# Intsights/PySubstringSearch

Measured on AMD Instinct MI355X. Metric: queries/sec (batched) + index-build GB/s on 512MB chunk, 1/2/4/8 GPU, higher is better.
Workload: dtype u64

## Files before the change

### include/pss.h

```cpp
#ifndef PSS_H
#define PSS_H

#include <stddef.h>
#include <stdint.h>

#ifdef __cplusplus
extern "C" {
#endif

#define PSS_OK 0
#define PSS_EINVAL (-1)
#define PSS_ENOMEM (-2)
#define PSS_EIO (-3)
#define PSS_ETOOBIG (-4)
#define PSS_EDEVICE (-5)
#define PSS_EFORMAT (-6)

typedef struct pss_writer pss_writer;
typedef struct pss_reader pss_reader;
typedef struct pss_result pss_result;


int pss_device_count(void);

// ... 233 lines not shown
    int (*send)(const void *buf, size_t count, int datatype, int peer, void *comm, void *stream);
    int (*recv)(void *buf, size_t count, int datatype, int peer, void *comm, void *stream);
    int (*all_gather)(const void *sendbuf, void *recvbuf, size_t sendcount, int datatype, void *comm, void *stream);
    const char *(*get_error_string)(int result);
} pss_rccl_api;
int pss_rccl_inject(const pss_rccl_api *api);
int pss_comm_adopt(void *nccl_comm, int32_t world, int32_t rank, int32_t device, pss_comm **out);

int pss_merge_packed(uint32_t world, uint64_t nq, const uint64_t *const *counts, const uint64_t *const *offsets,
                     const uint8_t *const *bytes, const uint64_t *num_entries, const uint64_t *num_bytes,
                     uint64_t *out_counts, uint64_t *out_offsets, uint8_t *out_bytes);
int pss_merge_packed_device(int32_t device, uint32_t world, uint64_t nq, const void *const *d_counts,
                            const void *const *d_starts, const void *const *d_bytes, const uint64_t *num_entries,
                            const uint64_t *num_bytes, void *d_out_counts, void *d_out_offsets, void *d_out_bytes);
int pss_reader_last_stats(const pss_reader *r, pss_search_stats *stats);
int pss_reader_close(pss_reader *r);

uint64_t pss_result_num_queries(const pss_result *res);
uint64_t pss_result_num_entries(const pss_result *res);
const uint64_t *pss_result_query_counts(const pss_result *res);
const uint64_t *pss_result_offsets(const pss_result *res);
const uint8_t *pss_result_bytes(const pss_result *res);
void pss_result_free(pss_result *res);


#define PSS_CORPUS_LINES 0
#define PSS_CORPUS_WORDS 1
#define PSS_CORPUS_RUNS 2
#define PSS_CORPUS_PERIODIC 3
#define PSS_CORPUS_REPEAT_LINE 4
// ... 10 lines not shown
```

### pysubstringsearch_amd/__init__.py

```python
import ctypes
import os
import typing

from . import _ffi
from ._ffi import lib as _lib

try:
    from . import _pssglue
except ImportError:
    _pssglue = None

__all__ = ['Writer', 'Reader', 'PackedResult', 'IdResult', 'DeviceResult', 'device_count', 'default_devices', 'release_workspace', 'workspace_bytes',
           'glob_parse', 'glob_escape', 'icase_variants']


def device_count() -> int:
    return _lib.pss_device_count()


def release_workspace() -> None:
    _ffi.check(_lib.pss_release_workspace())


def workspace_bytes(device: int = 0) -> int:
# ... 755 lines not shown
        import numpy as np
        nq = len(patterns)
        blob, offs = _pack_queries(patterns)
        counts = np.zeros(max(nq, 1), dtype=np.uint64)
        _ffi.check(_lib.pss_reader_count_batch(self._handle(), blob, offs.ctypes.data, nq, counts.ctypes.data))
        return [int(c) for c in counts[:nq]]

    def search_batch_raw(self, patterns: typing.Sequence[bytes]):
        return self._search_batch(patterns, False)

    def last_stats(self) -> dict:
        st = _ffi.SearchStats()
        _ffi.check(_lib.pss_reader_last_stats(self._handle(), ctypes.byref(st)))
        return st.as_dict()

    def search(self, substring: str) -> typing.List[str]:
        return self._search_batch([_utf8(substring, 'substring')], True)[0]

    def search_multiple(self, substrings: typing.List[str]) -> typing.List[str]:
        return self._search_batch([_utf8(s, 'substring') for s in substrings], True)[0]

    def close(self) -> None:
        if self._h:
            h, self._h = self._h, ctypes.c_void_p()
            _lib.pss_reader_close(h)

    def __enter__(self):
        return self

    def __exit__(self, *exc):
# ... 8 lines not shown
```

### pysubstringsearch_amd/_ffi.py

```python
import ctypes
import os

_HERE = os.path.dirname(os.path.abspath(__file__))
LIB_PATH = os.environ.get('PSS_LIBPSS') or os.path.join(_HERE, 'libpss.so')

PSS_OK, PSS_EINVAL, PSS_ENOMEM, PSS_EIO, PSS_ETOOBIG, PSS_EDEVICE, PSS_EFORMAT = 0, -1, -2, -3, -4, -5, -6

CORPUS_LINES, CORPUS_WORDS, CORPUS_RUNS, CORPUS_PERIODIC = 0, 1, 2, 3
CORPUS_REPEAT_LINE, CORPUS_DUP_BLOCKS, CORPUS_MIXED, CORPUS_SOURCE = 4, 5, 6, 7


class SaStats(ctypes.Structure):
    _fields_ = [
        ('sigma', ctypes.c_uint32),
        ('code_bits', ctypes.c_uint32),
        ('key_chars', ctypes.c_uint32),
        ('initial_passes', ctypes.c_uint32),
        ('rounds', ctypes.c_uint32),
        ('round_passes', ctypes.c_uint32),
        ('sum_active', ctypes.c_uint64),
        ('sort_elems', ctypes.c_uint64),
        ('ms_total', ctypes.c_double),
        ('ms_sort', ctypes.c_double),
        ('sort_launches', ctypes.c_uint64),
# ... 253 lines not shown
        'pss_reader_count_icase_batch': (ctypes.c_int, [vp, vp, vp, u32, vp]),
        'pss_icase_variants': (ctypes.c_int, [vp, u64, i32, vp, u64, ctypes.POINTER(u32), ctypes.POINTER(u32), ctypes.POINTER(u32)]),
        'pss_reader_chunk_entries': (ctypes.c_int, [vp, vp, vp, u64, ctypes.POINTER(u64)]),
        'pss_merge_packed': (ctypes.c_int, [u32, u64, vp, vp, vp, vp, vp, vp, vp, vp]),
        'pss_merge_packed_device': (ctypes.c_int, [i32, u32, u64, vp, vp, vp, vp, vp, vp, vp, vp]),
        'pss_comm_unique_id': (ctypes.c_int, [vp]),
        'pss_comm_init': (ctypes.c_int, [vp, i32, i32, i32, pvp]),
        'pss_comm_destroy': (ctypes.c_int, [vp]),
        'pss_gather_packed_rccl': (ctypes.c_int, [vp, ctypes.POINTER(DeviceResult), i32, pvp]),
        'pss_comm_set_timeout_ms': (ctypes.c_int, [vp, u32]),
        'pss_comm_status': (ctypes.c_int, [vp, ctypes.POINTER(u64), ctypes.POINTER(u64)]),
        'pss_rccl_inject': (ctypes.c_int, [ctypes.POINTER(RcclApiTable)]),
        'pss_comm_adopt': (ctypes.c_int, [vp, i32, i32, i32, pvp]),
        'pss_reload_env': (ctypes.c_int, []),
        'pss_reader_last_stats': (ctypes.c_int, [vp, ctypes.POINTER(SearchStats)]),
        'pss_reader_close': (ctypes.c_int, [vp]),
        'pss_result_num_queries': (u64, [vp]),
        'pss_result_num_entries': (u64, [vp]),
        'pss_result_query_counts': (ctypes.POINTER(u64), [vp]),
        'pss_result_offsets': (ctypes.POINTER(u64), [vp]),
        'pss_result_bytes': (ctypes.POINTER(ctypes.c_uint8), [vp]),
        'pss_result_free': (None, [vp]),
        'pss_gen_corpus': (ctypes.c_int, [ctypes.c_int, vp, u64, u64]),
    }
    for name, (res, args) in sig.items():
        fn = getattr(L, name)
        fn.restype = res
        fn.argtypes = args
    for what, have, want in (('pss_sa_stats', ctypes.sizeof(SaStats), L.pss_sa_stats_size()),
                             ('pss_search_stats', ctypes.sizeof(SearchStats), L.pss_search_stats_size())):
# ... 32 lines not shown
```

### pysubstringsearch_amd/csrc/capi.cpp

```cpp
#include <dlfcn.h>
#include <fcntl.h>
#include <sys/mman.h>
#include <sys/vfs.h>
#include <unistd.h>

#include <algorithm>
#include <atomic>
#include <cerrno>
#include <chrono>
#include <condition_variable>
#include <deque>
#include <mutex>
#include <string>
#include <thread>
#include <vector>

#include "common.h"
#include "radix_sort.h"
#include "sa_build.h"
#include "search.h"

using namespace pss;

namespace {
// ... 284 lines not shown
}

extern "C" int pss_reload_env(void)
{
    reload_search_knobs();
    return PSS_OK;
}

extern "C" int pss_reader_last_stats(const pss_reader *r, pss_search_stats *stats)
{
    if (!r || !stats) return PSS_EINVAL;
    *stats = r->last;
    return PSS_OK;
}

extern "C" int pss_reader_close(pss_reader *r)
{
    return guarded([&]() -> int {
        reader_free(r);
        return PSS_OK;
    });
}

extern "C" uint64_t pss_result_num_queries(const pss_result *res) { return res ? res->r.nq : 0; }
extern "C" uint64_t pss_result_num_entries(const pss_result *res) { return res ? res->r.n_entries : 0; }
extern "C" const uint64_t *pss_result_query_counts(const pss_result *res) { return res ? res->r.qcount : nullptr; }
extern "C" const uint64_t *pss_result_offsets(const pss_result *res) { return res ? res->r.offsets : nullptr; }
extern "C" const uint8_t *pss_result_bytes(const pss_result *res) { return res ? res->r.bytes : nullptr; }
extern "C" void pss_result_free(pss_result *res)
{
// ... 5 lines not shown
```

### pysubstringsearch_amd/csrc/capi_reader_impl.h

```cpp


struct pss_reader {
    int device = 0;
    DeviceCtx *ctx = nullptr;
    std::vector<ChunkDesc> chunks;
    struct Mem {
        void *text = nullptr;
        void *sa = nullptr;
        void *skeys = nullptr;
        bool sa_host = false;
        uint64_t hbm_bytes = 0, host_bytes = 0;
        void *lines = nullptr;
        uint64_t lines_bytes = 0;
        uint32_t line_shift = 0, entries = 0;
        bool lines_built = false;
    };
    std::vector<Mem> mem;
    std::vector<uint64_t> file_index;
    LineDesc *d_lines = nullptr;
    size_t d_lines_cap = 0;
    ChunkDesc *d_descs = nullptr;
    size_t d_descs_cap = 0;
    bool dirty = true;
    bool low_latency = false;
    bool order_sa = knob("PSS_RESULT_ORDER") != nullptr && strcmp(knob("PSS_RESULT_ORDER"), "sa") == 0;
    std::vector<uint64_t> heat, last_touch, batch_hits;
    std::vector<uint8_t> manual;
    uint64_t batch_seq = 0, auto_moves = 0;
    bool auto_residency = knob("PSS_READER_AUTO_RESIDENCY") == nullptr || atoi(knob("PSS_READER_AUTO_RESIDENCY")) != 0;
    pss_search_stats last{};
    struct Part;
    std::vector<Part *> parts;
    std::mutex multi_mu;
};

struct pss_reader::Part {
    pss_reader *reader = nullptr;
    std::thread worker;
    std::mutex mu;
    std::condition_variable cv;
    bool pending = false, quit = false;
    SearchRequest rq;
    int rc = 0;
    HostResult res;
    std::string err;
// ... 136 lines not shown
}

int multi_batch(pss_reader *r, const SearchRequest &rq, HostResult *out);

int reader_batch(pss_reader *r, SearchRequest rq, HostResult *res)
{
    if (!r->parts.empty()) return multi_batch(r, rq, res);
    std::lock_guard<std::recursive_mutex> lk(r->ctx->mu);
    PSS_HIP(hipSetDevice(r->device));
    PSS_TRY(reader_sync_descs(r));
    if (rq.mode == SEARCH_IDS) PSS_TRY(reader_ensure_lines(r));
    rq.sa_order = r->order_sa;
    rq.low_latency = r->low_latency && rq.mode == SEARCH_FULL && !rq.anchors && !rq.group_offsets;
    rq.chunk_hits = rq.mode == SEARCH_DEVICE ? nullptr : reader_hits_buffer(r);
    PSS_TRY(search_batch_device(r->ctx, r->d_descs, r->d_lines, (uint32_t)r->chunks.size(), rq, res, &r->last));
    reader_note_route(r);
    if (rq.chunk_hits) reader_note_batch(r);
    return PSS_OK;
}

void part_run(pss_reader::Part *p)
{
    p->res.release();
    p->err.clear();
    p->rc = reader_batch(p->reader, p->rq, &p->res);
    if (p->rc != PSS_OK) p->err = last_error();
}

void part_worker(pss_reader::Part *p)
{
// ... 415 lines not shown
        pss_reader::Part *p = r->parts[k];
        std::unique_lock<std::mutex> lk(p->mu);
        p->cv.wait(lk, [&] { return !p->pending; });
        if (p->rc != PSS_OK && rc == PSS_OK) {
            rc = p->rc;
            err = p->err;
        }
    }
    if (rc != PSS_OK) {
        set_error("%s", err.c_str());
        return rc;
    }
    pss_search_stats st{};
    st.queries = nq;
    uint64_t E = 0, B = 0;
    for (pss_reader::Part *p : r->parts) {
        const pss_search_stats &ps = p->reader->last;
        st.hits += ps.hits;
        st.entries += ps.entries;
        st.result_bytes += ps.result_bytes;
        st.ms_device = std::max(st.ms_device, ps.ms_device);
        st.ms_interval = std::max(st.ms_interval, ps.ms_interval);
        st.route |= ps.route;
        E += p->res.n_entries;
        B += p->res.n_bytes;
    }
    out->nq = nq;
    out->qcount = static_cast<uint64_t *>(calloc(nq ? nq : 1, sizeof(uint64_t)));
    if (!out->qcount) return PSS_ENOMEM;
    if (rq.mode == SEARCH_COUNTS) {
        for (pss_reader::Part *p : r->parts)
            for (uint32_t q = 0; q < nq; ++q) out->qcount[q] += p->res.qcount[q];
    } else {
        PSS_TRY(alloc_host_result(out, E, B, !search_knobs().no_pinned_results));
        struct RangeStart {
            uint32_t q0;
            uint64_t e_out, b_out;
            std::vector<uint64_t> cursor;
// ... 45 lines not shown
        };
        if (R == 1) {
            merge_range(0);
        } else {
            std::vector<std::thread> th;
            for (uint32_t i = 1; i < R; ++i) th.emplace_back(merge_range, i);
            merge_range(0);
            for (auto &t : th) t.join();
        }
        out->n_entries = E;
        out->n_bytes = B;
    }
    for (pss_reader::Part *p : r->parts) p->res.release();
    st.ms_host = std::chrono::duration<double, std::milli>(std::chrono::steady_clock::now() - t0).count();
    r->last = st;
    return PSS_OK;
}

int reader_batch_result(pss_reader *r, const SearchRequest &rq, pss_result **out)
{
    pss_result *res = new pss_result();
    const int rc = reader_batch(r, rq, &res->r);
    if (rc != PSS_OK) {
        pss_result_free(res);
        return rc;
    }
    *out = res;
    return PSS_OK;
}

// ... 938 lines not shown
```

### pysubstringsearch_amd/csrc/common.cpp

```cpp
#include "common.h"
#include "knobs.h"

#include <atomic>
#include <cstring>
#include <cstdio>
#include <cstdlib>
#include <algorithm>
#include <cerrno>
#include <unistd.h>

#include <mutex>
#include <vector>

namespace pss {

static thread_local std::string g_err;

void set_error(const char *fmt, ...)
{
    char buf[1024];
    va_list ap;
    va_start(ap, fmt);
    vsnprintf(buf, sizeof buf, fmt, ap);
    va_end(ap);
// ... 146 lines not shown
    std::unique_lock<std::mutex> lk(b->mu);
    b->cv.wait(lk, [&] { return b->finished == b->submitted; });
    return b->err;
}

void IoPool::wait_flag(Batch *b, std::atomic<int> *done)
{
    std::unique_lock<std::mutex> lk(b->mu);
    b->cv.wait(lk, [&] { return done->load(std::memory_order_acquire) != 0; });
}

int DeviceCtx::ensure_search_stage()
{
    if (search_stage) return PSS_OK;
    PSS_HIP(hipHostMalloc(&search_stage, kStageQ + kStageR, hipHostMallocDefault));
    return PSS_OK;
}

void SearchKnobs::load()
{
    *this = SearchKnobs{};
    no_small_path = knob("PSS_NO_SMALL_PATH") != nullptr;
    no_block_path = knob("PSS_NO_BLOCK_PATH") != nullptr;
    no_search_stage = knob("PSS_NO_SEARCH_STAGE") != nullptr;
    wave_search = knob("PSS_WAVE_SEARCH") != nullptr;
    no_group_search = knob("PSS_NO_GROUP_SEARCH") != nullptr;
    no_mid_pipeline = knob("PSS_NO_MID_PIPELINE") != nullptr;
    no_pinned_results = knob("PSS_NO_PINNED_RESULTS") != nullptr;
    small_path_events = knob("PSS_SEARCH_EVENTS") != nullptr;
    if (const char *e = knob("PSS_LANE_SEARCH_MIN")) lane_search_min = strtoull(e, nullptr, 0);
    if (const char *e = knob("PSS_ICASE_SEED_LETTERS")) icase_seed_letters = (uint32_t)std::min(6ul, std::max(1ul, strtoul(e, nullptr, 0)));
    if (const char *e = knob("PSS_RESIDENT_IDLE_US")) resident_idle_us = (uint32_t)strtoul(e, nullptr, 0);
    if (const char *e = knob("PSS_RESIDENT_LIFE_US")) resident_life_us = (uint32_t)strtoul(e, nullptr, 0);
}

static SearchKnobs g_knobs;
static std::once_flag g_knobs_once;
const SearchKnobs &search_knobs()
{
    std::call_once(g_knobs_once, []() { g_knobs.load(); });
    return g_knobs;
}
// ... 224 lines not shown
    {"PSS_WRITER_HOST_BUDGET", "8 GiB", "", "multi-device Writer: host text of the chunks in flight (one chunk always goes through)"},
    {"PSS_STRIPES", "8", "", "striped container format 2: stripe files of a Writer"},
    {"PSS_EXPERIMENT_NO_FILE", "unset", "", "measurement only: the record thread copies without writing the file"},
    {"PSS_RESULT_ORDER", "text", "sa", "Reader: 'sa' = the reference's order inside a chunk (suffix-array order of every entry's first hit)"},
    {"PSS_READER_HBM_BUDGET", "whatever hipMalloc grants minus 2 GiB", "", "Reader: suffix arrays beyond this many bytes of HBM stay in pinned host memory"},
    {"PSS_READER_AUTO_RESIDENCY", "1", "", "Reader: 0 = the residency manager never moves a suffix array by itself"},
    {"PSS_NO_KEY_SAMPLES", "unset", "", "Reader: no key-sample table"},
    {"PSS_SAMPLE_SHIFT", "11", "", "Reader: one key sample per 2^shift suffixes"},
    {"PSS_LINE_BLOCK_SHIFT", "8", "6|7|9|10", "Reader: the line index behind entry ids keeps one newline rank per 2^shift bytes of text (6 .. 10)"},
    {"PSS_NO_SMALL_PATH", "unset", "1", "search: no fused single-query kernels"},
    {"PSS_NO_BLOCK_PATH", "unset", "1", "search: small batches one wave per pair instead of one workgroup"},
    {"PSS_NO_SEARCH_STAGE", "unset", "1", "search: no pinned staging of queries and results"},
    {"PSS_WAVE_SEARCH", "unset", "1", "search: interval kernel one wave per pair at every batch size"},
    {"PSS_NO_GROUP_SEARCH", "unset", "1", "search: never 16 lanes per pair"},
    {"PSS_NO_MID_PIPELINE", "unset", "1", "search: always the general multi-kernel pipeline"},
    {"PSS_PINNED_POOL_BYTES", "40 GiB", "", "search: pinned host memory the result pool keeps between batches"},
    {"PSS_NO_PINNED_RESULTS", "unset", "1", "search: large results into pageable memory"},
    {"PSS_LANE_SEARCH_MIN", "8192", "1|100000", "search: pairs from which one lane per pair searches"},
    {"PSS_ICASE_SEED_LETTERS", "5", "1|2|3|4|5|6", "case-insensitive search: ASCII letters of a pattern's seed at most (2^letters spellings probed per pattern and chunk)"},
    {"PSS_SEARCH_EVENTS", "unset", "", "single-query path: HIP events around the fused kernel (fills ms_device; ~4 us per query)"},
    {"PSS_RESIDENT_IDLE_US", "1000", "", "low-latency mode: the resident kernel leaves after this long without a query"},
    {"PSS_RESIDENT_LIFE_US", "50000", "", "low-latency mode: ... and after this long in any case"},
    {"PSS_TRACE_RESIDENT", "unset", "", "libpss_trace.so only: print the resident kernel's phase stamps"},
    {"PSS_RCCL_LIB", "librccl.so of the process", "", "gather inside the C ABI: the RCCL library to load"},
    {"PSS_RCCL_TIMEOUT_MS", "60000", "", "gather inside the C ABI: bound of every wait for the peers"},
};
const int kNumKnobs = (int)(sizeof(kKnobs) / sizeof(kKnobs[0]));

const char *knob(const char *name)
{
// ... 48 lines not shown
```

### pysubstringsearch_amd/csrc/common.h

```cpp
#pragma once
#include <hip/hip_runtime.h>

#include <cstdarg>
#include <cstddef>
#include <cstdint>
#include <cstdio>
#include <cstdlib>
#include <cstring>
#include <atomic>
#include <condition_variable>
#include <deque>
#include <mutex>
#include <string>
#include <thread>
#include <vector>

#include "../../include/pss.h"

#include "knobs.h"

namespace pss {

void set_error(const char *fmt, ...);
const std::string &last_error();
// ... 16 lines not shown
struct DevBuf {
    void *p = nullptr;
    size_t cap = 0;
    int reserve(size_t bytes);
    void release();
    template <typename T> T *as() const { return static_cast<T *>(p); }
};

struct SearchKnobs {
    bool no_small_path = false;
    bool no_block_path = false;
    bool no_search_stage = false;
    bool wave_search = false;
    bool no_group_search = false;
    bool no_mid_pipeline = false;
    bool no_pinned_results = false;
    bool small_path_events = false;
    uint64_t lane_search_min = 8192;
    uint32_t icase_seed_letters = 5;
    uint32_t resident_idle_us = 1000;
    uint32_t resident_life_us = 50000;
    void load();
};
const SearchKnobs &search_knobs();
void reload_search_knobs();

void *pinned_pool_alloc(size_t bytes, size_t *granted);
void pinned_pool_free(void *p, size_t granted);
void pinned_pool_trim();

// ... 26 lines not shown
constexpr uint32_t kResidentStop = 0xffffffffu;

struct DeviceCtx {
    std::recursive_mutex mu;
    int device = -1;
    hipStream_t stream = nullptr;
    int num_cus = 256;
    static constexpr int kSlots = 57;
    DevBuf slot[kSlots];
    static constexpr size_t kPinnedBytes = (size_t)640 << 10;
    void *pinned = nullptr;
    size_t pinned_cap = 0;
    void *pinned_dev = nullptr;
    static constexpr size_t kStageQ = (size_t)2 << 20, kStageR = (size_t)4 << 20;
    void *search_stage = nullptr;
    int ensure_search_stage();
    hipEvent_t search_ev[3] = {nullptr, nullptr, nullptr};
    void *small_hdr_ready = nullptr;
    struct Resident {
        hipStream_t stream = nullptr;
        void *arena = nullptr, *arena_dev = nullptr;
        bool running = false;
        const void *chunks = nullptr;
        uint32_t nc = 0, spread = 0;
        void *d_arena = nullptr;
        uint32_t seq = 0;
        uint64_t launches = 0, served = 0, torn = 0;
        void post(const uint8_t *q, uint32_t plen);
    } resident;
    static constexpr size_t kResidentMailboxOff = 24576;
    int ensure_resident();
// ... 73 lines not shown
```

### pysubstringsearch_amd/csrc/search.hip

```cpp
#include "prims.h"
#include "scan.h"
#include "search.h"
#include "radix_sort.h"

#include <chrono>
#include <vector>

namespace pss {

constexpr u32 kSkip = 0xffffffffu;

struct InKept {
    const u32 *len;
    __device__ u64 operator()(u64 i) const { return len[i] != kSkip ? 1u : 0u; }
};
struct InLen {
    const u32 *len;
    __device__ u64 operator()(u64 i) const { const u32 l = len[i]; return l != kSkip ? l : 0u; }
};


__device__ __forceinline__ u64 load_text8(const u8 *p)
{
    const uintptr_t a = (uintptr_t)p;
// ... 1249 lines not shown
        const u64 o = boff[t];
        ent_off[eidx[t]] = o;
        copy_entry(out + o, ch.text + start[t], l);
    }
}

__global__ __launch_bounds__(256) void query_counts_kernel(u32 nc, u32 nq, const u64 *hit_off, const u64 *eidx,
                                                             u64 *qcount, const MidState *mid)
{
    const u32 q = blockIdx.x * blockDim.x + threadIdx.x;
    if (q >= nq || (mid && mid->flag)) return;
    const u64 v0 = (u64)q * nc, v1 = v0 + nc;
    qcount[q] = eidx[hit_off[v1]] - eidx[hit_off[v0]];
}


constexpr size_t SM_ARENA_RHDR = 64 + (size_t)SM_BYTE_CAP + 64;
constexpr size_t SM_ARENA_BYTES = SM_ARENA_RHDR + 64;
#if defined(__HIP_DEVICE_COMPILE__) && !defined(__gfx950__)
#error "search.hip is written for gfx950 (MI355X): the fused search kernels keep ~72 KiB of LDS per workgroup (160 KiB per CU there; gfx90a / gfx942 stop at 64 KiB)"
#endif

enum SSlot { Q_ORD_K0 = 50, Q_ORD_K1, Q_ORD_V0, Q_ORD_V1, Q_ORD_WORK, Q_BYTES = 10, Q_OFF, Q_LO, Q_CNT, Q_HITOFF, Q_START, Q_LEN, Q_EIDX, Q_BOFF, Q_ENTOFF, Q_OUT, Q_SMALL, Q_QCOUNT, Q_ANCHOR, Q_ARENA = 28, Q_HEAT = 46, Q_LINE_TMP = 47, Q_TERMS = 56 };

void HostResult::release()
{
    free(qcount);
    if (pinned) {
        pinned_pool_free(pinned, pinned_bytes);
    } else {
// ... 34 lines not shown
        const SmallRecord r = h_rec[ri];
        E += r.ent_count;
        for (u32 k = 0; k < r.ent_count; ++k) B += h_ent[r.ent_start + k].len;
    }
    std::vector<u8> h_more;
    const u8 *h_bytes = h_arena + SM_OFF_BYTES;
    if (B > SM_BYTE_PREFIX) {
        u8 *dst = nullptr;
        if (B <= DeviceCtx::kStageR && !knobs.no_search_stage && ctx->ensure_search_stage() == PSS_OK) {
            dst = static_cast<u8 *>(ctx->search_stage) + DeviceCtx::kStageQ;
        } else {
            h_more.resize(B);
            dst = h_more.data();
        }
        PSS_HIP(hipMemcpyAsync(dst, d_bytes, B, hipMemcpyDeviceToHost, s));
        PSS_HIP(hipStreamSynchronize(s));
        h_bytes = dst;
    }
    PSS_TRY(alloc_host_result(res, E, B, false));
    u64 e_out = 0, b_out = 0;
    for (u64 ri = 0; ri < nrec; ++ri) {
        const SmallRecord r = h_rec[ri];
        res->qcount[(ri / spread) / nc] += r.ent_count;
        if (chunk_hits) chunk_hits[(ri / spread) % nc] += r.ent_count;
        if (r.ent_count == 0) continue;
        const u64 first = b_out;
        for (u32 k = 0; k < r.ent_count; ++k) {
            res->offsets[e_out++] = b_out;
            b_out += h_ent[r.ent_start + k].len;
        }
// ... 200 lines not shown
        off_bytes = ((size_t)nq + 1) * 8;
        tiny = !anchored && qtotal + 32 <= 8192 && off_bytes <= 8192;
        const bool plain = !anchored && !terms && !sa_order;
        fused_ok = plain && rq.mode == SEARCH_FULL && tiny && nvq <= SM_MAX_VQ && !knobs.no_small_path;
        for (u32 i = 0; fused_ok && i < nq; ++i) fused_ok = rq.qoffsets[i + 1] - rq.qoffsets[i] <= SM_MAX_PLEN;
        resident_ok = fused_ok && rq.low_latency && nq == 1 && nvq <= SM_BLOCK_MAX_VQ && !knobs.no_block_path;
        mid_ok = plain && (rq.mode == SEARCH_FULL || device) && nvq <= MID_MAX && !knobs.no_mid_pipeline;
    }
    template <typename T>
    int take(SSlot which, size_t bytes, T *&p)
    {
        PSS_TRY(ctx->slot[which].reserve(bytes));
        p = ctx->slot[which].as<T>();
        return PSS_OK;
    }
    int stage_queries(), run_fused(bool *served), launch_interval(), run_mid(bool *done), pick_drivers(), union_spellings(), run_general(), finish();
    int sa_order_hits(u32 grid, u64 H);
    int download_result(u64 E, u64 B, const u64 *d_starts, const u8 *d_bytes, bool via_stage);
    void leave_on_device(const u64 *d_starts, const u8 *d_bytes), set_totals(u64 hits, u64 kept, u64 E, u64 B);
};

int empty_offsets(HostResult *res)
{
    res->offsets = (u64 *)calloc(1, sizeof(u64));
    return res->offsets ? PSS_OK : PSS_ENOMEM;
}

int empty_batch(DeviceCtx *ctx, const SearchRequest &rq, HostResult *res)
{
    if (rq.mode != SEARCH_DEVICE) return empty_offsets(res);
    if (rq.nq) {
        PSS_TRY(ctx->slot[Q_QCOUNT].reserve((size_t)rq.nq * 8));
        PSS_HIP(hipMemsetAsync(ctx->slot[Q_QCOUNT].p, 0, (size_t)rq.nq * 8, ctx->stream));
        PSS_HIP(hipStreamSynchronize(ctx->stream));
        res->d_qcount = ctx->slot[Q_QCOUNT].as<u64>();
    }
    return PSS_OK;
}

int Batch::stage_queries()
{
    PSS_TRY(take(Q_BYTES, qtotal + 32, d_q));
    PSS_TRY(take(Q_OFF, off_bytes, d_qoff));
    PSS_TRY(take(Q_LO, nvq * 4, d_lo));
    PSS_TRY(take(Q_CNT, nvq * 4, d_cnt));
    PSS_TRY(take(Q_HITOFF, (std::max(nvq, nrp) + 1) * 8, d_hitoff));
    PSS_TRY(take(Q_SMALL, SC_MAX_BLOCKS * 8 + 256, d_partial));
    PSS_TRY(take(Q_QCOUNT, (size_t)std::max(nq, nrow) * 8, d_qcount));
// ... 75 lines not shown
    SmallEntry *v_ent = reinterpret_cast<SmallEntry *>(v_arena + SM_OFF_ENT);
    const bool block_path = nvq <= SM_BLOCK_MAX_VQ && !knobs.no_block_path;
    u32 spread = 1;
    if (block_path)
        while (spread < SM_SPREAD && nvq * spread * 2 <= (nvq <= 32 ? 64u : 256u)) spread *= 2;
    st->route |= block_path ? PSS_ROUTE_SMALL_BLOCK : PSS_ROUTE_SMALL_WAVE;
    const u64 waves_per_block = 256 / kWave;
    if (block_path)
        hipLaunchKernelGGL(search_block_kernel, dim3((u32)nvq * spread), dim3(SM_BLOCK), 0, s, d_chunks, nc, v_q, v_qoff,
                           (u32)nvq, d_hdr, v_flags, v_rec, v_ent, d_bytes, v_arena + SM_OFF_BYTES, spread);
    else
        hipLaunchKernelGGL(search_small_kernel, dim3((u32)((nvq + waves_per_block - 1) / waves_per_block)), dim3(256),
                           0, s, d_chunks, nc, v_q, v_qoff, (u32)nvq, d_hdr, v_flags, v_rec, v_ent, d_bytes,
                           v_arena + SM_OFF_BYTES);
    if (timed) PSS_HIP(hipEventRecord(e2, s));
    PSS_HIP(hipStreamSynchronize(s));
    if (*h_overflow) {
        st->route |= PSS_ROUTE_SMALL_OVERFLOW;
        return PSS_OK;
    }
    PSS_TRY(small_collect(ctx, h_arena, d_bytes, nvq * spread, spread, nc, res, st, rq.chunk_hits));
    timed_route = timed;
    timed_interval = false;
    *served = true;
    return PSS_OK;
}

int Batch::launch_interval()
{
    if (h_padded) {
        PSS_HIP(hipMemcpyAsync(d_q, h_q, qtotal + 32, hipMemcpyHostToDevice, s));
// ... 16 lines not shown
                           d_qoff, nvq, d_lo, d_cnt);
    } else {
        st->route |= PSS_ROUTE_INTERVAL_WAVE;
        hipLaunchKernelGGL(search_interval_kernel, dim3((u32)((nvq + waves_per_block - 1) / waves_per_block)), dim3(256),
                           0, s, d_chunks, nc, d_q, d_qoff, nvq, d_lo, d_cnt);
    }
    PSS_HIP(hipEventRecord(e1, s));
    if (anchored)
        hipLaunchKernelGGL(anchor_edges_kernel, dim3((u32)((nvq + 255) / 256)), dim3(256), 0, s, d_chunks, nc, d_q, d_qoff,
                           d_aflags, nvq, d_cnt, d_edge);
    if (rq.chunk_hits && nc <= 4096) {
        PSS_TRY(ctx->slot[Q_HEAT].reserve((size_t)nc * 8));
        u64 *d_heat = ctx->slot[Q_HEAT].as<u64>();
        hipLaunchKernelGGL(chunk_hits_kernel, dim3(nc), dim3(256), 0, s, d_cnt, (u64)nq, nc, d_heat);
        PSS_HIP(hipMemcpyAsync(rq.chunk_hits, d_heat, (size_t)nc * 8, hipMemcpyDeviceToHost, s));
        PSS_HIP(hipStreamSynchronize(s));
    }
    return PSS_OK;
}

void Batch::leave_on_device(const u64 *d_starts, const u8 *d_bytes)
{
    res->d_qcount = d_qcount;
    res->d_offsets = d_starts;
    res->d_bytes = d_bytes;
}

int Batch::download_result(u64 E, u64 B, const u64 *d_starts, const u8 *d_bytes, bool via_stage)
{
    const size_t cnt_bytes = (size_t)nrow * 8;
    PSS_TRY(alloc_host_result(res, E, B, !via_stage && !knobs.no_pinned_results));
    u8 *to_off = reinterpret_cast<u8 *>(res->offsets), *to_bytes = res->bytes, *to_cnt = reinterpret_cast<u8 *>(res->qcount);
    const bool staged = via_stage && round_up(E * 8, 64) + round_up(B, 64) + cnt_bytes <= DeviceCtx::kStageR && !knobs.no_search_stage;
    if (staged) {
        PSS_TRY(ctx->ensure_search_stage());
        to_off = static_cast<u8 *>(ctx->search_stage) + DeviceCtx::kStageQ;
        to_bytes = to_off + round_up(E * 8, 64);
        to_cnt = to_bytes + round_up(B, 64);
    }
    if (E) PSS_HIP(hipMemcpyAsync(to_off, d_starts, E * 8, hipMemcpyDeviceToHost, s));
    if (B) PSS_HIP(hipMemcpyAsync(to_bytes, d_bytes, B, hipMemcpyDeviceToHost, s));
    PSS_HIP(hipMemcpyAsync(to_cnt, d_qcount, cnt_bytes, hipMemcpyDeviceToHost, s));
    PSS_HIP(hipStreamSynchronize(s));
    if (staged) {
        if (E) memcpy(res->offsets, to_off, E * 8);
        if (B) memcpy(res->bytes, to_bytes, B);
        memcpy(res->qcount, to_cnt, cnt_bytes);
    }
    res->offsets[E] = B;
    return PSS_OK;
}

void Batch::set_totals(u64 hits, u64 kept, u64 E, u64 B)
{
    res->n_entries = E;
    res->n_bytes = B;
    st->hits = hits;
    st->entries = kept;
// ... 7 lines not shown
    const u64 byte_cap = (u64)16 << 20;
    PSS_TRY(take(Q_START, (size_t)MID_MAX * 4, d_start));
    PSS_TRY(take(Q_LEN, (size_t)MID_MAX * 4, d_len));
    PSS_TRY(take(Q_EIDX, ((size_t)MID_MAX + 1) * 8, d_eidx));
    PSS_TRY(take(Q_BOFF, ((size_t)MID_MAX + 1) * 8, d_boff));
    PSS_TRY(take(Q_ENTOFF, ((size_t)MID_MAX + 1) * 8, d_entoff));
    PSS_TRY(take(Q_OUT, byte_cap + 16, d_out));
    MidState *d_ms = reinterpret_cast<MidState *>(d_total + 8);
    const u32 grid = (u32)ctx->num_cus * 4;
    hipLaunchKernelGGL(mid_hitoff_kernel, dim3(1), dim3(MID_BLOCK), 0, s, d_cnt, (u32)nvq, d_hitoff, d_ms);
    hipLaunchKernelGGL(hit_lines_kernel<false>, dim3(grid), dim3(256), 0, s, d_chunks, nc, d_q, d_qoff, nvq, d_lo, d_hitoff,
                       (u64)0, d_ms, d_start, d_len, (const u32 *)nullptr);
    hipLaunchKernelGGL(mid_hit_scans_kernel, dim3(1), dim3(MID_BLOCK), 0, s, d_len, d_ms, byte_cap, d_eidx, d_boff);
    hipLaunchKernelGGL(emit_kernel, dim3(grid), dim3(256), 0, s, d_chunks, nc, nvq, d_hitoff, (u64)0, d_ms, d_start,
                       d_len, d_eidx, d_boff, d_entoff, d_out);
    hipLaunchKernelGGL(query_counts_kernel, dim3((nq + 255) / 256), dim3(256), 0, s, nc, nq, d_hitoff, d_eidx, d_qcount,
                       (const MidState *)d_ms);
    PSS_HIP(hipEventRecord(e2, s));
    MidState *h_ms = reinterpret_cast<MidState *>(h_small);
    PSS_HIP(hipMemcpyAsync(h_ms, d_ms, sizeof(MidState), hipMemcpyDeviceToHost, s));
    PSS_HIP(hipStreamSynchronize(s));
    if (h_ms->flag) {
        st->route |= PSS_ROUTE_MID_OVERFLOW;
        return PSS_OK;
    }
    const u64 H = h_ms->hits, E = h_ms->entries, B = h_ms->bytes;
    if (device)
        leave_on_device(d_entoff, d_out);
    else
        PSS_TRY(download_result(E, B, d_entoff, d_out, true));
    set_totals(H, E, E, B);
    *done = true;
    return PSS_OK;
}

int Batch::sa_order_hits(u32 grid, u64 H)
{
    if (H >= (1ull << 32) || nvq >= (1ull << 33)) {
        set_error("search: %llu hits of %llu (query, chunk) pairs are more than the suffix-array result order takes in one batch",
                  (unsigned long long)H, (unsigned long long)nvq);
        return PSS_EINVAL;
    }
    u64 *OK[2];
    u32 *OV[2];
    PSS_TRY(take(Q_ORD_K0, H * 8, OK[0]));
// ... 47 lines not shown
    PSS_HIP(hipMemcpyAsync(d_foff, rq.fold_offsets, ((size_t)nrow + 1) * 8, hipMemcpyHostToDevice, s));
    PSS_HIP(hipMemcpyAsync(d_fseed, rq.fold_seed, (size_t)nrow * 4, hipMemcpyHostToDevice, s));
    PSS_HIP(hipMemcpyAsync(d_fvoid, own_tflags.data(), nrow, hipMemcpyHostToDevice, s));
    PSS_HIP(hipMemsetAsync(d_fbytes + ftotal, 0, 32, s));
    PSS_HIP(hipMemcpyAsync(d_fbytes, rq.fold_bytes, ftotal, hipMemcpyHostToDevice, s));
    hipLaunchKernelGGL(fold_union_kernel, dim3((u32)((nrp + 255) / 256)), dim3(256), 0, s, nc, d_goff, d_fvoid, d_cnt, nrp, p_cnt);
    return PSS_OK;
}

int Batch::run_general()
{
    st->route |= PSS_ROUTE_GENERAL | (sa_order ? PSS_ROUTE_SA_ORDER : 0u) | (counts ? PSS_ROUTE_COUNTS : 0u) |
                   (anchored ? PSS_ROUTE_ANCHORED : 0u);
    PSS_TRY(device_excl_scan(ctx, InU32{p_cnt}, nrp, d_partial, d_total, d_hitoff));
    PSS_HIP(hipMemcpyAsync(h_small, d_total, 8, hipMemcpyDeviceToHost, s));
    PSS_HIP(hipStreamSynchronize(s));
    const u64 H = h_small[0];
    if (H == 0) {
        PSS_HIP(hipEventRecord(e2, s));
        if (device) {
            PSS_HIP(hipMemsetAsync(d_qcount, 0, (size_t)nrow * 8, s));
            leave_on_device(nullptr, nullptr);
        }
        PSS_HIP(hipStreamSynchronize(s));
        if (!device) PSS_TRY(empty_offsets(res));
        set_totals(0, 0, 0, 0);
        return PSS_OK;
    }
    PSS_TRY(take(Q_START, H * 4, d_start));
    PSS_TRY(take(Q_LEN, H * 4, d_len));
    PSS_TRY(take(Q_EIDX, (H + 1) * 8, d_eidx));
    PSS_TRY(take(Q_BOFF, (H + 1) * 8, d_boff));
    const u32 grid = (u32)std::min<u64>((u64)ctx->num_cus * 16, (H + 255) / 256);
    if (sa_order)
        PSS_TRY(sa_order_hits(grid, H));
    else if (anchored)
        hipLaunchKernelGGL(anchored_hits_kernel, dim3(grid), dim3(256), 0, s, d_chunks, nc, d_aflags, nrp, p_lo, d_edge,
                           d_hitoff, H, d_start, d_len);
    else if (fold) {
// ... 11 lines not shown
            hipLaunchKernelGGL(seq_verify_kernel, dim3(vgrid), dim3(256), 0, s, d_chunks, nc, d_q, d_qoff, d_goff, d_sanch, nrp,
                               d_hitoff, H, d_start, d_len);
        else
            hipLaunchKernelGGL(terms_verify_kernel, dim3(vgrid), dim3(256), 0, s, d_chunks, nc, d_q, d_qoff, d_goff, d_tflags, d_cnt,
                               d_gdrv, nrp, d_hitoff, H, d_start, d_len);
    } else
        hipLaunchKernelGGL(hit_lines_kernel<false>, dim3(grid), dim3(256), 0, s, d_chunks, nc, d_q, d_qoff, nrp, p_lo,
                           d_hitoff, H, (const MidState *)nullptr, d_start, d_len, (const u32 *)nullptr);
    PSS_TRY(device_excl_scan(ctx, InKept{d_len}, H, d_partial, d_total, d_eidx));
    PSS_HIP(hipMemcpyAsync(h_small, d_total, 8, hipMemcpyDeviceToHost, s));
    if (counts) {
        hipLaunchKernelGGL(query_counts_kernel, dim3((nrow + 255) / 256), dim3(256), 0, s, nc, nrow, d_hitoff, d_eidx,
                           d_qcount, (const MidState *)nullptr);
        PSS_HIP(hipEventRecord(e2, s));
        PSS_HIP(hipMemcpyAsync(res->qcount, d_qcount, (size_t)nrow * 8, hipMemcpyDeviceToHost, s));
        PSS_HIP(hipStreamSynchronize(s));
        PSS_TRY(empty_offsets(res));
        set_totals(H, h_small[0], 0, 0);
        return PSS_OK;
    }
    if (!ids) {
        PSS_TRY(device_excl_scan(ctx, InLen{d_len}, H, d_partial, d_total, d_boff));
        PSS_HIP(hipMemcpyAsync(h_small + 1, d_total, 8, hipMemcpyDeviceToHost, s));
    }
    PSS_HIP(hipStreamSynchronize(s));
    const u64 E = h_small[0], B = ids ? E * 8 : h_small[1];
    PSS_TRY(take(Q_ENTOFF, (E + 1) * 8, d_entoff));
    PSS_TRY(take(Q_OUT, B + 16, d_out));
    if (ids)
        hipLaunchKernelGGL(emit_ids_kernel, dim3(grid), dim3(256), 0, s, d_chunks, d_lines, nc, nrp, d_hitoff, H, d_start, d_len,
                           d_eidx, d_entoff, reinterpret_cast<u64 *>(d_out));
    else
        hipLaunchKernelGGL(emit_kernel, dim3(grid), dim3(256), 0, s, d_chunks, nc, nrp, d_hitoff, H,
                           (const MidState *)nullptr, d_start, d_len, d_eidx, d_boff, d_entoff, d_out);
    hipLaunchKernelGGL(query_counts_kernel, dim3((nrow + 255) / 256), dim3(256), 0, s, nc, nrow, d_hitoff, d_eidx,
                       d_qcount, (const MidState *)nullptr);
    PSS_HIP(hipEventRecord(e2, s));
    if (device) {
        leave_on_device(d_entoff, d_out);
        PSS_HIP(hipStreamSynchronize(s));
    } else {
        PSS_TRY(download_result(E, B, d_entoff, d_out, false));
    }
    set_totals(H, E, E, B);
    return PSS_OK;
}

int Batch::finish()
{
    PSS_HIP(hipGetLastError());
    float ms = 0.f;
    if (timed_route) {
        PSS_HIP(hipEventElapsedTime(&ms, e0, e2));
        st->ms_device = st->ms_interval = ms;
    }
// ... 17 lines not shown
        return PSS_EINVAL;
    }
    if (rq.anchors && (rq.mode == SEARCH_DEVICE || rq.low_latency)) {
        set_error("search: an anchored batch takes the general pipeline to a host result");
        return PSS_EINVAL;
    }
    if (rq.group_offsets && (rq.anchors || (rq.nq && !rq.exclude && !rq.seq_anchors && !rq.fold_seed) || rq.mode == SEARCH_DEVICE || rq.low_latency)) {
        set_error("search: an all-terms batch takes the general pipeline to a host result, and its terms are not anchored");
        return PSS_EINVAL;
    }
    if (rq.fold_seed && (!rq.group_offsets || !rq.fold_bytes || !rq.fold_offsets || rq.exclude || rq.seq_anchors)) {
        set_error("search: a case-insensitive batch is the spellings of its patterns' seeds in groups, without exclusions or anchors");
        return PSS_EINVAL;
    }
    const u32 rows = rq.rows();
    memset(st, 0, sizeof *st);
    st->queries = rows;
    res->nq = rows;
    res->qcount = (u64 *)calloc(rows ? rows : 1, sizeof(u64));
    res->offsets = nullptr;
    res->bytes = nullptr;
    res->n_entries = 0;
    if (!res->qcount) return PSS_ENOMEM;
    if (rows == 0 || rq.nq == 0 || nc == 0) return empty_batch(ctx, rq, res);

    Batch b(ctx, d_chunks, d_lines, nc, rq, res, st);
    PSS_TRY(b.stage_queries());
    if (b.fused_ok) {
        bool served = false;
        PSS_TRY(b.run_fused(&served));
// ... 169 lines not shown
```

Baseline: 71.47.

## Deliver mid-pipeline results to pinned host stage from device, skipping second wait

Adds a mid_deliver_kernel that computes per-query counts and writes the header, counts, entry offsets and result bytes straight into the pinned host staging buffer through its device pointer. The host then needs one stream wait and plain memcpys instead of a header download, a wait, and then separate async copies with a second wait. This removes a host-device round trip per mid-size batch, at the cost of many small PCIe writes issued by the kernel and a size cap set by the stage buffer. It also adds a stream-wait counter exposed through the API, plus a knob that disables delivery.

After: 71.40. Within noise of the previous version (-0.1%).

```diff
diff --git a/include/pss.h b/include/pss.h
--- a/include/pss.h
+++ b/include/pss.h
@@ -271,6 +271,7 @@
                             const void *const *d_starts, const void *const *d_bytes, const uint64_t *num_entries,
                             const uint64_t *num_bytes, void *d_out_counts, void *d_out_offsets, void *d_out_bytes);
 int pss_reader_last_stats(const pss_reader *r, pss_search_stats *stats);
+uint32_t pss_reader_last_stream_waits(const pss_reader *r);
 int pss_reader_close(pss_reader *r);
 
 uint64_t pss_result_num_queries(const pss_result *res);
diff --git a/pysubstringsearch_amd/__init__.py b/pysubstringsearch_amd/__init__.py
--- a/pysubstringsearch_amd/__init__.py
+++ b/pysubstringsearch_amd/__init__.py
@@ -793,6 +793,9 @@
         _ffi.check(_lib.pss_reader_last_stats(self._handle(), ctypes.byref(st)))
         return st.as_dict()
 
+    def last_stream_waits(self) -> int:
+        return int(_lib.pss_reader_last_stream_waits(self._handle()))
+
     def search(self, substring: str) -> typing.List[str]:
         return self._search_batch([_utf8(substring, 'substring')], True)[0]
 
diff --git a/pysubstringsearch_amd/_ffi.py b/pysubstringsearch_amd/_ffi.py
--- a/pysubstringsearch_amd/_ffi.py
+++ b/pysubstringsearch_amd/_ffi.py
@@ -291,6 +291,7 @@
         'pss_comm_adopt': (ctypes.c_int, [vp, i32, i32, i32, pvp]),
         'pss_reload_env': (ctypes.c_int, []),
         'pss_reader_last_stats': (ctypes.c_int, [vp, ctypes.POINTER(SearchStats)]),
+        'pss_reader_last_stream_waits': (u32, [vp]),
         'pss_reader_close': (ctypes.c_int, [vp]),
         'pss_result_num_queries': (u64, [vp]),
         'pss_result_num_entries': (u64, [vp]),
diff --git a/pysubstringsearch_amd/csrc/capi.cpp b/pysubstringsearch_amd/csrc/capi.cpp
--- a/pysubstringsearch_amd/csrc/capi.cpp
+++ b/pysubstringsearch_amd/csrc/capi.cpp
@@ -322,6 +322,8 @@
     return PSS_OK;
 }
 
+extern "C" uint32_t pss_reader_last_stream_waits(const pss_reader *r) { return r ? r->last_waits : 0; }
+
 extern "C" int pss_reader_close(pss_reader *r)
 {
     return guarded([&]() -> int {
diff --git a/pysubstringsearch_amd/csrc/capi_reader_impl.h b/pysubstringsearch_amd/csrc/capi_reader_impl.h
--- a/pysubstringsearch_amd/csrc/capi_reader_impl.h
+++ b/pysubstringsearch_amd/csrc/capi_reader_impl.h
@@ -29,6 +29,7 @@
     uint64_t batch_seq = 0, auto_moves = 0;
     bool auto_residency = knob("PSS_READER_AUTO_RESIDENCY") == nullptr || atoi(knob("PSS_READER_AUTO_RESIDENCY")) != 0;
     pss_search_stats last{};
+    uint32_t last_waits = 0;
     struct Part;
     std::vector<Part *> parts;
     std::mutex multi_mu;
@@ -195,6 +196,7 @@
     rq.low_latency = r->low_latency && rq.mode == SEARCH_FULL && !rq.anchors && !rq.group_offsets;
     rq.chunk_hits = rq.mode == SEARCH_DEVICE ? nullptr : reader_hits_buffer(r);
     PSS_TRY(search_batch_device(r->ctx, r->d_descs, r->d_lines, (uint32_t)r->chunks.size(), rq, res, &r->last));
+    r->last_waits = r->ctx->search_waits;
     reader_note_route(r);
     if (rq.chunk_hits) reader_note_batch(r);
     return PSS_OK;
@@ -640,6 +642,7 @@
     pss_search_stats st{};
     st.queries = nq;
     uint64_t E = 0, B = 0;
+    uint32_t waits = 0;
     for (pss_reader::Part *p : r->parts) {
         const pss_search_stats &ps = p->reader->last;
         st.hits += ps.hits;
@@ -648,6 +651,7 @@
         st.ms_device = std::max(st.ms_device, ps.ms_device);
         st.ms_interval = std::max(st.ms_interval, ps.ms_interval);
         st.route |= ps.route;
+        waits = std::max(waits, p->reader->last_waits);
         E += p->res.n_entries;
         B += p->res.n_bytes;
     }
@@ -723,6 +727,7 @@
     for (pss_reader::Part *p : r->parts) p->res.release();
     st.ms_host = std::chrono::duration<double, std::milli>(std::chrono::steady_clock::now() - t0).count();
     r->last = st;
+    r->last_waits = waits;
     return PSS_OK;
 }
 
diff --git a/pysubstringsearch_amd/csrc/common.cpp b/pysubstringsearch_amd/csrc/common.cpp
--- a/pysubstringsearch_amd/csrc/common.cpp
+++ b/pysubstringsearch_amd/csrc/common.cpp
@@ -184,6 +184,7 @@
 {
     if (search_stage) return PSS_OK;
     PSS_HIP(hipHostMalloc(&search_stage, kStageQ + kStageR, hipHostMallocDefault));
+    PSS_HIP(hipHostGetDevicePointer(&search_stage_dev, search_stage, 0));
     return PSS_OK;
 }
 
@@ -196,6 +197,7 @@
     wave_search = knob("PSS_WAVE_SEARCH") != nullptr;
     no_group_search = knob("PSS_NO_GROUP_SEARCH") != nullptr;
     no_mid_pipeline = knob("PSS_NO_MID_PIPELINE") != nullptr;
+    no_mid_deliver = knob("PSS_MID_NO_DELIVER") != nullptr;
     no_pinned_results = knob("PSS_NO_PINNED_RESULTS") != nullptr;
     small_path_events = knob("PSS_SEARCH_EVENTS") != nullptr;
     if (const char *e = knob("PSS_LANE_SEARCH_MIN")) lane_search_min = strtoull(e, nullptr, 0);
@@ -450,6 +452,7 @@
     {"PSS_WAVE_SEARCH", "unset", "1", "search: interval kernel one wave per pair at every batch size"},
     {"PSS_NO_GROUP_SEARCH", "unset", "1", "search: never 16 lanes per pair"},
     {"PSS_NO_MID_PIPELINE", "unset", "1", "search: always the general multi-kernel pipeline"},
+    {"PSS_MID_NO_DELIVER", "unset", "1", "search: the mid pipeline's result is fetched by the host (copies and a second wait) instead of delivered by the device"},
     {"PSS_PINNED_POOL_BYTES", "40 GiB", "", "search: pinned host memory the result pool keeps between batches"},
     {"PSS_NO_PINNED_RESULTS", "unset", "1", "search: large results into pageable memory"},
     {"PSS_LANE_SEARCH_MIN", "8192", "1|100000", "search: pairs from which one lane per pair searches"},
diff --git a/pysubstringsearch_amd/csrc/common.h b/pysubstringsearch_amd/csrc/common.h
--- a/pysubstringsearch_amd/csrc/common.h
+++ b/pysubstringsearch_amd/csrc/common.h
@@ -54,6 +54,7 @@
     bool wave_search = false;
     bool no_group_search = false;
     bool no_mid_pipeline = false;
+    bool no_mid_deliver = false;
     bool no_pinned_results = false;
     bool small_path_events = false;
     uint64_t lane_search_min = 8192;
@@ -110,7 +111,9 @@
     void *pinned_dev = nullptr;
     static constexpr size_t kStageQ = (size_t)2 << 20, kStageR = (size_t)4 << 20;
     void *search_stage = nullptr;
+    void *search_stage_dev = nullptr;
     int ensure_search_stage();
+    uint32_t search_waits = 0;
     hipEvent_t search_ev[3] = {nullptr, nullptr, nullptr};
     void *small_hdr_ready = nullptr;
     struct Resident {
diff --git a/pysubstringsearch_amd/csrc/search.hip b/pysubstringsearch_amd/csrc/search.hip
--- a/pysubstringsearch_amd/csrc/search.hip
+++ b/pysubstringsearch_amd/csrc/search.hip
@@ -1287,6 +1287,56 @@
     qcount[q] = eidx[hit_off[v1]] - eidx[hit_off[v0]];
 }
 
+constexpr size_t MID_HDR = 64;
+__host__ __device__ inline u64 mid_round64(u64 x) { return (x + 63) & ~(u64)63; }
+__host__ __device__ inline u64 mid_payload_bytes(u64 nq, u64 E, u64 B)
+{
+    return MID_HDR + mid_round64(nq * 8) + mid_round64((E + 1) * 8) + mid_round64(B);
+}
+
+__global__ __launch_bounds__(256) void mid_deliver_kernel(u32 nc, u32 nq, const u64 *hit_off, const u64 *eidx, u64 *qcount,
+                                                            const MidState *ms, const u64 *ent_off, const u8 *bytes, u8 *stage,
+                                                            u64 cap)
+{
+    const u64 tid = (u64)blockIdx.x * blockDim.x + threadIdx.x, nthreads = (u64)gridDim.x * blockDim.x;
+    const u32 flag = ms->flag;
+    const u64 H = ms->hits, E = ms->entries, B = ms->bytes;
+    const bool deliver = !flag && mid_payload_bytes(nq, E, B) <= cap;
+    if (tid == 0) {
+        MidState line = {H, E, B, flag, deliver ? 1u : 0u};
+        *reinterpret_cast<MidState *>(stage) = line;
+    }
+    if (flag) return;
+    uint4 *s_cnt = reinterpret_cast<uint4 *>(stage + MID_HDR);
+    const u64 cnt_units = mid_round64((u64)nq * 8) / 16;
+    for (u64 i = tid; i < cnt_units; i += nthreads) {
+        u64 c[2] = {0, 0};
+        for (u32 k = 0; k < 2; ++k) {
+            const u64 q = 2 * i + k;
+            if (q < nq) {
+                c[k] = eidx[hit_off[(q + 1) * nc]] - eidx[hit_off[q * nc]];
+                qcount[q] = c[k];
+            }
+        }
+        if (deliver) s_cnt[i] = make_uint4((u32)c[0], (u32)(c[0] >> 32), (u32)c[1], (u32)(c[1] >> 32));
+    }
+    if (!deliver) return;
+    uint4 *s_off = s_cnt + cnt_units;
+    const u64 off_units = mid_round64((E + 1) * 8) / 16;
+    for (u64 i = tid; i < off_units; i += nthreads) {
+        u64 o[2];
+        for (u32 k = 0; k < 2; ++k) {
+            const u64 e = 2 * i + k;
+            o[k] = e < E ? ent_off[e] : (e == E ? B : 0);
+        }
+        s_off[i] = make_uint4((u32)o[0], (u32)(o[0] >> 32), (u32)o[1], (u32)(o[1] >> 32));
+    }
+    uint4 *s_bytes = s_off + off_units;
+    const uint4 *src = reinterpret_cast<const uint4 *>(bytes);
+    const u64 byte_units = mid_round64(B) / 16;
+    for (u64 i = tid; i < byte_units; i += nthreads) s_bytes[i] = src[i];
+}
+
 
 constexpr size_t SM_ARENA_RHDR = 64 + (size_t)SM_BYTE_CAP + 64;
 constexpr size_t SM_ARENA_BYTES = SM_ARENA_RHDR + 64;
@@ -1351,6 +1401,7 @@
             dst = h_more.data();
         }
         PSS_HIP(hipMemcpyAsync(dst, d_bytes, B, hipMemcpyDeviceToHost, s));
+        ++ctx->search_waits;
         PSS_HIP(hipStreamSynchronize(s));
         h_bytes = dst;
     }
@@ -1581,6 +1632,12 @@
         p = ctx->slot[which].as<T>();
         return PSS_OK;
     }
+    int wait()
+    {
+        ++ctx->search_waits;
+        PSS_HIP(hipStreamSynchronize(s));
+        return PSS_OK;
+    }
     int stage_queries(), run_fused(bool *served), launch_interval(), run_mid(bool *done), pick_drivers(), union_spellings(), run_general(), finish();
     int sa_order_hits(u32 grid, u64 H);
     int download_result(u64 E, u64 B, const u64 *d_starts, const u8 *d_bytes, bool via_stage);
@@ -1599,6 +1656,7 @@
     if (rq.nq) {
         PSS_TRY(ctx->slot[Q_QCOUNT].reserve((size_t)rq.nq * 8));
         PSS_HIP(hipMemsetAsync(ctx->slot[Q_QCOUNT].p, 0, (size_t)rq.nq * 8, ctx->stream));
+        ++ctx->search_waits;
         PSS_HIP(hipStreamSynchronize(ctx->stream));
         res->d_qcount = ctx->slot[Q_QCOUNT].as<u64>();
     }
@@ -1704,7 +1762,7 @@
                            0, s, d_chunks, nc, v_q, v_qoff, (u32)nvq, d_hdr, v_flags, v_rec, v_ent, d_bytes,
                            v_arena + SM_OFF_BYTES);
     if (timed) PSS_HIP(hipEventRecord(e2, s));
-    PSS_HIP(hipStreamSynchronize(s));
+    PSS_TRY(wait());
     if (*h_overflow) {
         st->route |= PSS_ROUTE_SMALL_OVERFLOW;
         return PSS_OK;
@@ -1751,7 +1809,7 @@
         u64 *d_heat = ctx->slot[Q_HEAT].as<u64>();
         hipLaunchKernelGGL(chunk_hits_kernel, dim3(nc), dim3(256), 0, s, d_cnt, (u64)nq, nc, d_heat);
         PSS_HIP(hipMemcpyAsync(rq.chunk_hits, d_heat, (size_t)nc * 8, hipMemcpyDeviceToHost, s));
-        PSS_HIP(hipStreamSynchronize(s));
+        PSS_TRY(wait());
     }
     return PSS_OK;
 }
@@ -1778,7 +1836,7 @@
     if (E) PSS_HIP(hipMemcpyAsync(to_off, d_starts, E * 8, hipMemcpyDeviceToHost, s));
     if (B) PSS_HIP(hipMemcpyAsync(to_bytes, d_bytes, B, hipMemcpyDeviceToHost, s));
     PSS_HIP(hipMemcpyAsync(to_cnt, d_qcount, cnt_bytes, hipMemcpyDeviceToHost, s));
-    PSS_HIP(hipStreamSynchronize(s));
+    PSS_TRY(wait());
     if (staged) {
         if (E) memcpy(res->offsets, to_off, E * 8);
         if (B) memcpy(res->bytes, to_bytes, B);
@@ -1816,21 +1874,40 @@
     hipLaunchKernelGGL(mid_hit_scans_kernel, dim3(1), dim3(MID_BLOCK), 0, s, d_len, d_ms, byte_cap, d_eidx, d_boff);
     hipLaunchKernelGGL(emit_kernel, dim3(grid), dim3(256), 0, s, d_chunks, nc, nvq, d_hitoff, (u64)0, d_ms, d_start,
                        d_len, d_eidx, d_boff, d_entoff, d_out);
-    hipLaunchKernelGGL(query_counts_kernel, dim3((nq + 255) / 256), dim3(256), 0, s, nc, nq, d_hitoff, d_eidx, d_qcount,
-                       (const MidState *)d_ms);
-    PSS_HIP(hipEventRecord(e2, s));
-    MidState *h_ms = reinterpret_cast<MidState *>(h_small);
-    PSS_HIP(hipMemcpyAsync(h_ms, d_ms, sizeof(MidState), hipMemcpyDeviceToHost, s));
-    PSS_HIP(hipStreamSynchronize(s));
+    const bool deliver = !device && !knobs.no_search_stage && !knobs.no_mid_deliver && ctx->ensure_search_stage() == PSS_OK;
+    const MidState *h_ms = reinterpret_cast<const MidState *>(h_small);
+    const u8 *h_stage = nullptr;
+    if (deliver) {
+        h_stage = static_cast<const u8 *>(ctx->search_stage) + DeviceCtx::kStageQ;
+        h_ms = reinterpret_cast<const MidState *>(h_stage);
+        hipLaunchKernelGGL(mid_deliver_kernel, dim3((u32)ctx->num_cus), dim3(256), 0, s, nc, nq, d_hitoff, d_eidx, d_qcount,
+                           (const MidState *)d_ms, d_entoff, d_out, static_cast<u8 *>(ctx->search_stage_dev) + DeviceCtx::kStageQ,
+                           (u64)DeviceCtx::kStageR);
+        PSS_HIP(hipEventRecord(e2, s));
+    } else {
+        hipLaunchKernelGGL(query_counts_kernel, dim3((nq + 255) / 256), dim3(256), 0, s, nc, nq, d_hitoff, d_eidx, d_qcount,
+                           (const MidState *)d_ms);
+        PSS_HIP(hipEventRecord(e2, s));
+        PSS_HIP(hipMemcpyAsync(h_small, d_ms, sizeof(MidState), hipMemcpyDeviceToHost, s));
+    }
+    PSS_TRY(wait());
     if (h_ms->flag) {
         st->route |= PSS_ROUTE_MID_OVERFLOW;
         return PSS_OK;
     }
     const u64 H = h_ms->hits, E = h_ms->entries, B = h_ms->bytes;
-    if (device)
+    if (device) {
         leave_on_device(d_entoff, d_out);
-    else
+    } else if (deliver && h_ms->pad) {
+        const u8 *from_cnt = h_stage + MID_HDR, *from_off = from_cnt + mid_round64((u64)nq * 8);
+        const u8 *from_bytes = from_off + mid_round64((E + 1) * 8);
+        PSS_TRY(alloc_host_result(res, E, B, false));
+        memcpy(res->qcount, from_cnt, (size_t)nq * 8);
+        memcpy(res->offsets, from_off, (size_t)(E + 1) * 8);
+        if (B) memcpy(res->bytes, from_bytes, (size_t)B);
+    } else {
         PSS_TRY(download_result(E, B, d_entoff, d_out, true));
+    }
     set_totals(H, E, E, B);
     *done = true;
     return PSS_OK;
@@ -1908,7 +1985,7 @@
                    (anchored ? PSS_ROUTE_ANCHORED : 0u);
     PSS_TRY(device_excl_scan(ctx, InU32{p_cnt}, nrp, d_partial, d_total, d_hitoff));
     PSS_HIP(hipMemcpyAsync(h_small, d_total, 8, hipMemcpyDeviceToHost, s));
-    PSS_HIP(hipStreamSynchronize(s));
+    PSS_TRY(wait());
     const u64 H = h_small[0];
     if (H == 0) {
         PSS_HIP(hipEventRecord(e2, s));
@@ -1916,7 +1993,7 @@
             PSS_HIP(hipMemsetAsync(d_qcount, 0, (size_t)nrow * 8, s));
             leave_on_device(nullptr, nullptr);
         }
-        PSS_HIP(hipStreamSynchronize(s));
+        PSS_TRY(wait());
         if (!device) PSS_TRY(empty_offsets(res));
         set_totals(0, 0, 0, 0);
         return PSS_OK;
@@ -1958,7 +2035,7 @@
                            d_qcount, (const MidState *)nullptr);
         PSS_HIP(hipEventRecord(e2, s));
         PSS_HIP(hipMemcpyAsync(res->qcount, d_qcount, (size_t)nrow * 8, hipMemcpyDeviceToHost, s));
-        PSS_HIP(hipStreamSynchronize(s));
+        PSS_TRY(wait());
         PSS_TRY(empty_offsets(res));
         set_totals(H, h_small[0], 0, 0);
         return PSS_OK;
@@ -1967,7 +2044,7 @@
         PSS_TRY(device_excl_scan(ctx, InLen{d_len}, H, d_partial, d_total, d_boff));
         PSS_HIP(hipMemcpyAsync(h_small + 1, d_total, 8, hipMemcpyDeviceToHost, s));
     }
-    PSS_HIP(hipStreamSynchronize(s));
+    PSS_TRY(wait());
     const u64 E = h_small[0], B = ids ? E * 8 : h_small[1];
     PSS_TRY(take(Q_ENTOFF, (E + 1) * 8, d_entoff));
     PSS_TRY(take(Q_OUT, B + 16, d_out));
@@ -1982,7 +2059,7 @@
     PSS_HIP(hipEventRecord(e2, s));
     if (device) {
         leave_on_device(d_entoff, d_out);
-        PSS_HIP(hipStreamSynchronize(s));
+        PSS_TRY(wait());
     } else {
         PSS_TRY(download_result(E, B, d_entoff, d_out, false));
     }
@@ -2030,6 +2107,7 @@
         return PSS_EINVAL;
     }
     const u32 rows = rq.rows();
+    ctx->search_waits = 0;
     memset(st, 0, sizeof *st);
     st->queries = rows;
     res->nq = rows;
```
